# SEAME-pt/Team02-ObjectDetection

Hardware: NVIDIA B200
Metric: MobileNetV2UNet inference images/s (higher is better)
Workload: dtype bf16

## Files before the change

### include/b200seg.h

```cpp
#ifndef B200SEG_H_
#define B200SEG_H_

#include <stdint.h>

#ifdef __cplusplus
extern "C" {
#endif

typedef struct CUstream_st* b200seg_stream_t;

enum { B200SEG_F32 = 0, B200SEG_BF16 = 1 };
enum { B200SEG_ACT_NONE = 0, B200SEG_ACT_RELU = 1, B200SEG_ACT_RELU6 = 2 };

int b200seg_version(void);
const char* b200seg_last_error(void);
int b200seg_device_info(int* sm_count, int* cc);

int b200seg_conv3x3_smallcin(const void* x, int x_dtype, const float* w, const float* b, void* y,
                             int y_dtype, int B, int Cin, int H, int W, int Cout, int stride, int act,
                             b200seg_stream_t s);

int b200seg_stem_mb1_supported(int x_dtype, int H, int W, int Cstem, int Cout);
int b200seg_stem_mb1(const void* x, int x_dtype, const float* w_stem, const float* b_stem, const void* w_dw,
                     const float* b_dw, const void* w_pw, const float* b_pw, void* y, int B, int H, int W,
                     b200seg_stream_t s);

int b200seg_dwconv3x3(const void* x, const float* w, const float* b, void* y, int dtype, int B, int H,
                      int W, int C, int stride, int act, b200seg_stream_t s);

int b200seg_dwconv3x3_bf16w(const void* x, const void* w, const float* b, void* y, int B, int H, int W, int C, int stride,
                            int act, int variant, b200seg_stream_t s);

int b200seg_conv_tc(const void* x, const void* w, const float* b, const void* res, void* y, int B, int H,
                    int W, int Cin, int Cout, int taps, int act, int flags, b200seg_stream_t s);

int b200seg_conv_rs_supported(int H, int W, int Cin, int Cout);
int b200seg_conv_rs(const void* x, const void* w, const float* b, const void* res, void* y, int B, int H, int W, int Cin,
                    int Cout, int act, int flags, b200seg_stream_t s);

int b200seg_dwconv3x3_tc(const void* x, const void* wdiag, const float* b, void* y, int B, int H, int W,
                         int C, int stride, int act, int flags, b200seg_stream_t s);

int b200seg_conv_simt(const void* x, const float* w, const float* b, const void* res, void* y, int dtype,
                      int B, int H, int W, int Cin, int Cout, int taps, int act, b200seg_stream_t s);

int b200seg_upsample2x_concat(const void* skip, const void* x, void* y, int dtype, int B, int h, int w,
                              int Cs, int Cu, b200seg_stream_t s);

int b200seg_upsample2x_ac_nchw(const void* logits, int dtype, int ldc, void* out, int out_dtype, int B,
                               int h, int w, int C, b200seg_stream_t s);
int b200seg_upsample2x_ac_argmax(const void* logits, int dtype, int ldc, uint8_t* mask, int B, int h,
                                 int w, int C, b200seg_stream_t s);

int b200seg_mbconv(const void* x, const void* w_exp, const float* b_exp, const void* w_dw, const float* b_dw,
                   const void* w_proj, const float* b_proj, int residual, void* y, int B, int H, int W, int Cin,
                   int Ce, int Cout, int stride, int flags, b200seg_stream_t s);

int b200seg_tail_fused(const void* x, const void* w0, const float* b0, const void* w3, const float* b3, void* out,
                       int out_dtype, uint8_t* mask, int B, int h, int w, int C, b200seg_stream_t s);

int b200seg_nhwc_to_nchw(const void* x, int dtype, int ldc, void* out, int out_dtype, int B, int H, int W,
                         int C, b200seg_stream_t s);

int b200seg_maxpool2x2(const void* x, void* y, int dtype, int B, int H, int W, int C, b200seg_stream_t s);

int b200seg_softmax_ce(const float* logits, const int64_t* target, float* loss_sum, float* dlogits,
                       float grad_scale, const float* counts, int B, int C, int H, int W, b200seg_stream_t s);
int b200seg_scale_unless_one(float* x, long long n, const float* s, b200seg_stream_t st);
int b200seg_ce_count(const int64_t* target, float* counts, long long N, int C, long long ignore_index,
                     b200seg_stream_t s);

int b200seg_upsample2x_ac_generic(const void* logits, int dtype, int ldc, void* out, int out_dtype, uint8_t* mask, int B,
                                  int h, int w, int C, b200seg_stream_t s);
int b200seg_final_bwd_generic(const float* dout, void* dlogits, int dtype, int B, int h, int w, int C, int ldc,
                              b200seg_stream_t s);
int b200seg_nhwc_argmax(const void* x, int dtype, int ldc, uint8_t* mask, long long P, int C, b200seg_stream_t s);

int b200seg_bn_stats(const void* z, int dtype, long long P, int C, double* sum, double* sumsq, int nslot,
                     long long slot_stride, b200seg_stream_t s);
int b200seg_bn_finalize(const void* z, int dtype, const double* sum, const double* sumsq, int nslot,
                        long long slot_stride, long long n, const float* gamma,
                        const float* beta, float eps, float momentum, float* running_mean, float* running_var,
                        float* mean, float* invstd, float* scale, float* shift, int C, b200seg_stream_t s);
int b200seg_bn_apply(const void* z, const float* scale, const float* shift, const void* res, void* a, int dtype,
                     long long P, int C, int act, b200seg_stream_t s);
int b200seg_bn_finalize_apply(const void* z, const double* st_sums, int nslot, const float* gamma, const float* beta, float eps,
                              float momentum, float* running_mean, float* running_var, float* sv, const void* res, void* a,
                              int dtype, long long P, int C, int act, b200seg_stream_t s);
int b200seg_bn_bwd_reduce(const void* da, const void* z, const float* scale, const float* shift, const float* mean,
                          const float* invstd, int dtype, long long P, int C, int act, double* sg, double* sgx,
                          int nslot, long long slot_stride, b200seg_stream_t s);
int b200seg_bn_bwd_apply(const void* da, const void* z, const float* scale, const float* shift, const float* mean,
                         const float* invstd, const float* sg, const float* sgx, void* dz, int dtype, long long P,
                         int C, int act, b200seg_stream_t s);
int b200seg_bn_bwd_apply_slots(const void* da, const void* z, const float* sv, const double* red, int nslot, void* dz,
                               int dtype, long long P, int C, int act, b200seg_stream_t s);
int b200seg_bn_cluster_supported(int dtype, long long P, int C);
int b200seg_bn_cluster_bwd_supported(int dtype, long long P, int C);
int b200seg_bn_cluster_fwd(const void* z, long long P, int C, const float* gamma, const float* beta, float eps, float momentum,
                           float* running_mean, float* running_var, float* sv, const void* res, void* a, int act,
                           b200seg_stream_t s);
int b200seg_bn_cluster_bwd(const void* da, const void* z, const float* sv, long long P, int C, int act, double* red, void* dz,
                           b200seg_stream_t s);
int b200seg_act_bwd(const void* da, const void* a_out, void* dz, int dtype, long long N, int act, b200seg_stream_t s);
int b200seg_colsum(const void* x, int dtype, long long P, int C, double* out, int nslot, long long slot_stride,
                   b200seg_stream_t s);
int b200seg_f64_to_f32(const double* in, float* out, int n, int nslot, long long slot_stride, float scale,
                       b200seg_stream_t s);
int b200seg_conv_wgrad(const void* x, const void* dz, float* dw, int dtype, int B, int H, int W, int Cin, int Cout,
                       int taps, b200seg_stream_t s);
int b200seg_conv_wgrad_tc(const void* x, const void* dz, float* dw, int B, int H, int W, int Cin, int Cout, int taps,
                          b200seg_stream_t s);
int b200seg_dw_dgrad(const void* dz, const float* w, const void* acc_in, void* dx, int dtype, int B, int H, int W,
                     int C, int stride, b200seg_stream_t s);
int b200seg_dw_wgrad(const void* x, const void* dz, double* dw, int nslot, int dtype, int B, int H, int W, int C,
                     int stride, b200seg_stream_t s);
int b200seg_smallcin_wgrad(const void* x, int x_dtype, const void* dz, int dtype, float* dw, int B, int Cin, int H,
                           int W, int Cout, int stride, b200seg_stream_t s);
int b200seg_upcat_bwd(const void* dcat, const void* acc_skip, void* dskip, void* dx, int dtype, int B, int h, int w,
                      int Cs, int Cu, b200seg_stream_t s);
int b200seg_final_bwd(const float* dout, void* dlogits, int dtype, int B, int h, int w, int C, b200seg_stream_t s);
int b200seg_nchw_to_nhwc_pad(const float* x, void* y, int dtype, int B, int C, int H, int W, int ldc,
                             b200seg_stream_t s);
int b200seg_maxpool_bwd(const void* x, const void* dy, const void* acc_in, void* dx, int dtype, int B, int H, int W,
                        int C, b200seg_stream_t s);

int b200seg_adam_multi(const void* table, const int* chunk_tensor, const int* chunk_index, int n_chunks, float lr,
                       double one_minus_beta1, float beta2, double one_minus_beta2, float eps, float weight_decay,
                       double bias_corr1, double bias_corr2, b200seg_stream_t s);
int b200seg_adam_chunk(void);
int b200seg_pack_weights_multi(const void* table, const int* chunk_tensor, const int* chunk_index, int n_chunks,
                               b200seg_stream_t s);
int b200seg_pack_chunk(void);
int b200seg_fold_pack_eval_multi(const void* table, const int* chunk_tensor, const int* chunk_index, int n_chunks,
                                 b200seg_stream_t s);
int b200seg_fold_chunk(void);
int b200seg_grad_finalize_multi(const void* table, const int* chunk_tensor, const int* chunk_index, int n_chunks,
                                b200seg_stream_t s);
int b200seg_grad_chunk(void);

int b200seg_preprocess_u8(const uint8_t* frames, int B, int Hs, int Ws, void* out, int out_dtype, uint8_t* rgb, int H,
                          int W, float mean0, float mean1, float mean2, float std0, float std1, float std2,
                          b200seg_stream_t s);

int b200seg_remap_labels(const uint8_t* in, int64_t* out, const uint8_t* lut256, long long n, b200seg_stream_t s);

#ifdef __cplusplus
}
#endif
#endif
```

### team02-objectdetection_b200/b200seg/_cabi.py

```python
from __future__ import annotations

import ctypes as C
import os

_HERE = os.path.dirname(os.path.abspath(__file__))
LIB_PATH = os.path.join(_HERE, "libb200seg.so")

F32, BF16 = 0, 1
ACT_NONE, ACT_RELU, ACT_RELU6 = 0, 1, 2

_vp, _i, _f, _ll, _d = C.c_void_p, C.c_int, C.c_float, C.c_longlong, C.c_double

_PROTOS = {
    "b200seg_version": [],
    "b200seg_device_info": [C.POINTER(_i), C.POINTER(_i)],
    "b200seg_conv3x3_smallcin": [_vp, _i, _vp, _vp, _vp, _i, _i, _i, _i, _i, _i, _i, _i, _vp],
    "b200seg_stem_mb1_supported": [_i, _i, _i, _i, _i],
    "b200seg_stem_mb1": [_vp, _i, _vp, _vp, _vp, _vp, _vp, _vp, _vp, _i, _i, _i, _vp],
    "b200seg_dwconv3x3": [_vp, _vp, _vp, _vp, _i, _i, _i, _i, _i, _i, _i, _vp],
    "b200seg_dwconv3x3_bf16w": [_vp, _vp, _vp, _vp, _i, _i, _i, _i, _i, _i, _i, _vp],
    "b200seg_conv_tc": [_vp, _vp, _vp, _vp, _vp, _i, _i, _i, _i, _i, _i, _i, _i, _vp],
    "b200seg_conv_rs_supported": [_i, _i, _i, _i],
    "b200seg_conv_rs": [_vp, _vp, _vp, _vp, _vp, _i, _i, _i, _i, _i, _i, _i, _vp],
    "b200seg_dwconv3x3_tc": [_vp, _vp, _vp, _vp, _i, _i, _i, _i, _i, _i, _i, _vp],
    "b200seg_mbconv": [_vp, _vp, _vp, _vp, _vp, _vp, _vp, _i, _vp, _i, _i, _i, _i, _i, _i, _i, _i, _vp],
    "b200seg_conv_simt": [_vp, _vp, _vp, _vp, _vp, _i, _i, _i, _i, _i, _i, _i, _i, _vp],
    "b200seg_upsample2x_concat": [_vp, _vp, _vp, _i, _i, _i, _i, _i, _i, _vp],
    "b200seg_upsample2x_ac_nchw": [_vp, _i, _i, _vp, _i, _i, _i, _i, _i, _vp],
    "b200seg_upsample2x_ac_argmax": [_vp, _i, _i, _vp, _i, _i, _i, _i, _vp],
    "b200seg_tail_fused": [_vp, _vp, _vp, _vp, _vp, _vp, _i, _vp, _i, _i, _i, _i, _vp],
    "b200seg_nhwc_to_nchw": [_vp, _i, _i, _vp, _i, _i, _i, _i, _i, _vp],
    "b200seg_maxpool2x2": [_vp, _vp, _i, _i, _i, _i, _i, _vp],
    "b200seg_softmax_ce": [_vp, _vp, _vp, _vp, _f, _vp, _i, _i, _i, _i, _vp],
    "b200seg_scale_unless_one": [_vp, _ll, _vp, _vp],
    "b200seg_remap_labels": [_vp, _vp, _vp, _ll, _vp],
    "b200seg_ce_count": [_vp, _vp, _ll, _i, _ll, _vp],
    "b200seg_upsample2x_ac_generic": [_vp, _i, _i, _vp, _i, _vp, _i, _i, _i, _i, _vp],
    "b200seg_final_bwd_generic": [_vp, _vp, _i, _i, _i, _i, _i, _i, _vp],
    "b200seg_nhwc_argmax": [_vp, _i, _i, _vp, _ll, _i, _vp],
    "b200seg_bn_stats": [_vp, _i, _ll, _i, _vp, _vp, _i, _ll, _vp],
    "b200seg_bn_finalize": [_vp, _i, _vp, _vp, _i, _ll, _ll, _vp, _vp, _f, _f, _vp, _vp, _vp, _vp, _vp, _vp, _i, _vp],
    "b200seg_bn_apply": [_vp, _vp, _vp, _vp, _vp, _i, _ll, _i, _i, _vp],
    "b200seg_bn_bwd_reduce": [_vp, _vp, _vp, _vp, _vp, _vp, _i, _ll, _i, _i, _vp, _vp, _i, _ll, _vp],
    "b200seg_bn_cluster_supported": [_i, _ll, _i],
    "b200seg_bn_cluster_bwd_supported": [_i, _ll, _i],
    "b200seg_bn_cluster_fwd": [_vp, _ll, _i, _vp, _vp, _f, _f, _vp, _vp, _vp, _vp, _vp, _i, _vp],
    "b200seg_bn_cluster_bwd": [_vp, _vp, _vp, _ll, _i, _i, _vp, _vp, _vp],
    "b200seg_bn_bwd_apply": [_vp, _vp, _vp, _vp, _vp, _vp, _vp, _vp, _vp, _i, _ll, _i, _i, _vp],
    "b200seg_bn_bwd_apply_slots": [_vp, _vp, _vp, _vp, _i, _vp, _i, _ll, _i, _i, _vp],
    "b200seg_bn_finalize_apply": [_vp, _vp, _i, _vp, _vp, _f, _f, _vp, _vp, _vp, _vp, _vp, _i, _ll, _i, _i, _vp],
    "b200seg_act_bwd": [_vp, _vp, _vp, _i, _ll, _i, _vp],
    "b200seg_colsum": [_vp, _i, _ll, _i, _vp, _i, _ll, _vp],
    "b200seg_f64_to_f32": [_vp, _vp, _i, _i, _ll, _f, _vp],
    "b200seg_conv_wgrad": [_vp, _vp, _vp, _i, _i, _i, _i, _i, _i, _i, _vp],
    "b200seg_conv_wgrad_tc": [_vp, _vp, _vp, _i, _i, _i, _i, _i, _i, _vp],
    "b200seg_dw_dgrad": [_vp, _vp, _vp, _vp, _i, _i, _i, _i, _i, _i, _vp],
    "b200seg_dw_wgrad": [_vp, _vp, _vp, _i, _i, _i, _i, _i, _i, _i, _vp],
    "b200seg_smallcin_wgrad": [_vp, _i, _vp, _i, _vp, _i, _i, _i, _i, _i, _i, _vp],
    "b200seg_upcat_bwd": [_vp, _vp, _vp, _vp, _i, _i, _i, _i, _i, _i, _vp],
    "b200seg_final_bwd": [_vp, _vp, _i, _i, _i, _i, _i, _vp],
    "b200seg_nchw_to_nhwc_pad": [_vp, _vp, _i, _i, _i, _i, _i, _i, _vp],
    "b200seg_preprocess_u8": [_vp, _i, _i, _i, _vp, _i, _vp, _i, _i, _f, _f, _f, _f, _f, _f, _vp],
    "b200seg_adam_multi": [_vp, _vp, _vp, _i, _f, _d, _f, _d, _f, _f, _d, _d, _vp],
    "b200seg_adam_chunk": [],
    "b200seg_pack_weights_multi": [_vp, _vp, _vp, _i, _vp],
    "b200seg_pack_chunk": [],
    "b200seg_fold_pack_eval_multi": [_vp, _vp, _vp, _i, _vp],
    "b200seg_fold_chunk": [],
    "b200seg_grad_finalize_multi": [_vp, _vp, _vp, _i, _vp],
    "b200seg_grad_chunk": [],
    "b200seg_maxpool_bwd": [_vp, _vp, _vp, _vp, _i, _i, _i, _i, _i, _vp],
}
EXPORTS = sorted(list(_PROTOS) + ["b200seg_last_error"])


def _load():
    if not os.path.exists(LIB_PATH):
        raise ImportError(
            f"{LIB_PATH} not found: build it with `python team02-objectdetection_b200/build.py` "
            "(nvcc, sm_100a). b200seg has no CPU/eager fallback.")
    lib = C.CDLL(LIB_PATH)
    for name, args in _PROTOS.items():
        fn = getattr(lib, name)
        fn.argtypes = args
        fn.restype = _i
    lib.b200seg_last_error.argtypes = []
    lib.b200seg_last_error.restype = C.c_char_p
    return lib


lib = _load()


LAUNCHES = [0]


def check(rc: int, what: str = "") -> None:
    LAUNCHES[0] += 1
    if rc != 0:
        msg = lib.b200seg_last_error().decode("utf-8", "replace")
        raise RuntimeError(f"libb200seg {what} failed (rc={rc}): {msg}")


def ptr(t) -> int:
    return 0 if t is None else t.data_ptr()


def device_info():
    sm, cc = _i(0), _i(0)
    check(lib.b200seg_device_info(C.byref(sm), C.byref(cc)), "device_info")
    return sm.value, cc.value
```

### team02-objectdetection_b200/b200seg/ops.py

```python
from __future__ import annotations

from typing import Optional

import os

import torch

from . import _cabi
from ._cabi import ACT_NONE, ACT_RELU, ACT_RELU6, BF16, F32, check, lib, ptr

_DT = {torch.float32: F32, torch.bfloat16: BF16}


def _dt(t: torch.Tensor) -> int:
    try:
        return _DT[t.dtype]
    except KeyError:
        raise TypeError(f"b200seg supports float32 and bfloat16 activations, got {t.dtype}") from None


def _cuda(*ts):
    for t in ts:
        if t is None:
            continue
        if not t.is_cuda:
            raise RuntimeError("b200seg ops need CUDA tensors (no CPU fallback)")
        if not t.is_contiguous():
            raise RuntimeError("b200seg ops need contiguous tensors")


def _stream() -> int:
    return torch.cuda.current_stream().cuda_stream


_MUTATION_EPOCH = 0


def mutation_epoch() -> int:
    return _MUTATION_EPOCH


def bump_mutation_epoch() -> None:
    global _MUTATION_EPOCH
    _MUTATION_EPOCH += 1


def conv3x3_smallcin(x_nchw, w, b, stride: int, act: int, out_dtype, out=None):
    _cuda(x_nchw, w, b)
    B, Cin, H, W = x_nchw.shape
    Cout = w.shape[-1]
    Ho, Wo = (H - 1) // stride + 1, (W - 1) // stride + 1
    if out is None:
        out = torch.empty((B, Ho, Wo, Cout), device=x_nchw.device, dtype=out_dtype)
    check(lib.b200seg_conv3x3_smallcin(ptr(x_nchw), _dt(x_nchw), ptr(w), ptr(b), ptr(out), _dt(out), B, Cin, H, W,
                                       Cout, stride, act, _stream()), "conv3x3_smallcin")
    return out


def stem_mb1_supported(x_nchw, cstem: int, cout: int) -> bool:
    return bool(lib.b200seg_stem_mb1_supported(_dt(x_nchw), x_nchw.shape[2], x_nchw.shape[3], cstem, cout))


def stem_mb1(x_nchw, w_stem, b_stem, w_dw, b_dw, w_pw, b_pw, out=None):
    _cuda(x_nchw, w_stem, b_stem, w_dw, b_dw, w_pw, b_pw)
    B, C, H, W = x_nchw.shape
    if C != 3 or not x_nchw.is_contiguous():
        raise ValueError("stem_mb1 expects a contiguous NCHW tensor with 3 channels")
    if w_dw.dtype != torch.bfloat16 or w_pw.dtype != torch.bfloat16 or w_stem.dtype != torch.float32:
        raise TypeError("stem_mb1: w_stem f32, w_dw / w_pw bf16")
    if out is None:
        out = torch.empty((B, H // 2, W // 2, w_pw.shape[0]), device=x_nchw.device, dtype=torch.bfloat16)
    check(lib.b200seg_stem_mb1(ptr(x_nchw), _dt(x_nchw), ptr(w_stem), ptr(b_stem), ptr(w_dw), ptr(b_dw), ptr(w_pw), ptr(b_pw),
                               ptr(out), B, H, W, _stream()), "stem_mb1")
    return out


def dwconv3x3(x, w9c, b, stride: int, act: int, out=None):
    _cuda(x, w9c, b)
    B, H, W, Cc = x.shape
    Ho, Wo = (H - 1) // stride + 1, (W - 1) // stride + 1
    if out is None:
        out = torch.empty((B, Ho, Wo, Cc), device=x.device, dtype=x.dtype)
    check(lib.b200seg_dwconv3x3(ptr(x), ptr(w9c), ptr(b), ptr(out), _dt(x), B, H, W, Cc, stride, act, _stream()),
          "dwconv3x3")
    return out


def dwconv3x3_bf16w(x, w9c_bf16, b, stride: int, act: int, out=None, variant: int = 0):
    _cuda(x, w9c_bf16, b)
    if x.dtype != torch.bfloat16 or w9c_bf16.dtype != torch.bfloat16:
        raise TypeError("dwconv3x3_bf16w is bf16-only")
    B, H, W, Cc = x.shape
    if tuple(w9c_bf16.shape) != (9, Cc):
        raise ValueError(f"dwconv3x3_bf16w: taps {tuple(w9c_bf16.shape)} != (9, {Cc})")
    Ho, Wo = (H - 1) // stride + 1, (W - 1) // stride + 1
    if out is None:
        out = torch.empty((B, Ho, Wo, Cc), device=x.device, dtype=torch.bfloat16)
    check(lib.b200seg_dwconv3x3_bf16w(ptr(x), ptr(w9c_bf16), ptr(b), ptr(out), B, H, W, Cc, stride, act, variant, _stream()),
          "dwconv3x3_bf16w")
    return out


def pack_dw_diag(w9c: torch.Tensor) -> torch.Tensor:
    C = w9c.shape[1]
    out = torch.zeros(C, 9, 64, device=w9c.device, dtype=torch.bfloat16)
    idx = torch.arange(C, device=w9c.device)
    out[idx, :, idx % 64] = w9c.t().to(torch.bfloat16)
    return out.contiguous()


def dwconv3x3_tc(x, wdiag, b, stride: int, act: int, out=None, flags: int = 0):
    _cuda(x, wdiag, b)
    if x.dtype != torch.bfloat16 or wdiag.dtype != torch.bfloat16:
        raise TypeError("dwconv3x3_tc is bf16-only")
    B, H, W, Cc = x.shape
    if tuple(wdiag.shape) != (Cc, 9, 64):
        raise ValueError(f"dwconv3x3_tc: wdiag {tuple(wdiag.shape)} != ({Cc}, 9, 64)")
    Ho, Wo = (H - 1) // stride + 1, (W - 1) // stride + 1
    if out is None:
        out = torch.empty((B, Ho, Wo, Cc), device=x.device, dtype=torch.bfloat16)
    check(lib.b200seg_dwconv3x3_tc(ptr(x), ptr(wdiag), ptr(b), ptr(out), B, H, W, Cc, stride, act, flags, _stream()),
          "dwconv3x3_tc")
    return out


USE_CONV_RS = True
CONV_RS_FLAGS = 0


def conv_rs(x, w, b, act: int, res=None, out=None, flags: int = 0):
    _cuda(x, w, b, res)
    if x.dtype != torch.bfloat16 or w.dtype != torch.bfloat16:
        raise TypeError("conv_rs is bf16-only")
    B, H, W, Cin = x.shape
    Cout = w.shape[0]
    if w.shape[1] != 9 * Cin:
        raise ValueError(f"conv_rs: weight {tuple(w.shape)} does not match Cin={Cin}")
    if out is None:
        out = torch.empty((B, H, W, Cout), device=x.device, dtype=torch.bfloat16)
    check(lib.b200seg_conv_rs(ptr(x), ptr(w), ptr(b), ptr(res), ptr(out), B, H, W, Cin, Cout, act, flags, _stream()), "conv_rs")
    return out


def conv_tc(x, w, b, taps: int, act: int, res=None, out=None, flags: int = 0):
    _cuda(x, w, b, res)
    if x.dtype != torch.bfloat16 or w.dtype != torch.bfloat16:
        raise TypeError("conv_tc is bf16-only")
    B, H, W, Cin = x.shape
    Cout = w.shape[0]
    if w.shape[1] != taps * Cin:
        raise ValueError(f"conv_tc: weight {tuple(w.shape)} does not match taps={taps} Cin={Cin}")
    if (taps == 9 and USE_CONV_RS and flags == 0 and lib.b200seg_conv_rs_supported(H, W, Cin, Cout)
            and (Cout <= 32 or res is None)):
        return conv_rs(x, w, b, act, res, out, CONV_RS_FLAGS)
    if out is None:
        out = torch.empty((B, H, W, Cout), device=x.device, dtype=torch.bfloat16)
    check(lib.b200seg_conv_tc(ptr(x), ptr(w), ptr(b), ptr(res), ptr(out), B, H, W, Cin, Cout, taps, act, flags,
                              _stream()), "conv_tc")
    return out


def conv_simt(x, w, b, taps: int, act: int, res=None, out=None):
    _cuda(x, w, b, res)
    if w.dtype != torch.float32:
        raise TypeError("conv_simt weights are f32")
    B, H, W, Cin = x.shape
    Cout = w.shape[0]
    if w.shape[1] != taps * Cin:
        raise ValueError(f"conv_simt: weight {tuple(w.shape)} does not match taps={taps} Cin={Cin}")
    if out is None:
        out = torch.empty((B, H, W, Cout), device=x.device, dtype=x.dtype)
    check(lib.b200seg_conv_simt(ptr(x), ptr(w), ptr(b), ptr(res), ptr(out), _dt(x), B, H, W, Cin, Cout, taps, act,
                                _stream()), "conv_simt")
    return out


def pad_channels(t: torch.Tensor, mult: int) -> torch.Tensor:
    c = t.shape[-1]
    cp = (c + mult - 1) // mult * mult
    if cp == c:
        return t.contiguous()
    out = torch.zeros((*t.shape[:-1], cp), device=t.device, dtype=t.dtype)
    out[..., :c] = t
    return out


def mbconv(x, w_exp, b_exp, w_dw, b_dw, w_proj, b_proj, stride: int, residual: bool, out=None, flags: int = 0):
    _cuda(x, w_exp, b_exp, w_dw, b_dw, w_proj, b_proj)
    if x.dtype != torch.bfloat16 or w_exp.dtype != torch.bfloat16 or w_proj.dtype != torch.bfloat16 or w_dw.dtype != torch.bfloat16:
        raise TypeError("mbconv is bf16-only (activations, 1x1 weights and depthwise taps)")
    B, H, W, Cin = x.shape
    Ce, Cout = w_exp.shape[0], w_proj.shape[0]
    cep, cop = (Ce + 63) // 64 * 64, (Cout + 15) // 16 * 16
    if (tuple(w_exp.shape) != (Ce, Cin) or tuple(w_proj.shape) != (Cout, Ce) or tuple(w_dw.shape) != (9, cep)
            or b_exp.numel() != cep or b_dw.numel() != cep or b_proj.numel() != cop):
        raise ValueError(f"mbconv: operand shapes w_exp {tuple(w_exp.shape)} w_dw {tuple(w_dw.shape)} "
                         f"w_proj {tuple(w_proj.shape)} b {b_exp.numel()},{b_dw.numel()},{b_proj.numel()}")
    Ho, Wo = (H - 1) // stride + 1, (W - 1) // stride + 1
    if out is None:
        out = torch.empty((B, Ho, Wo, Cout), device=x.device, dtype=torch.bfloat16)
    check(lib.b200seg_mbconv(ptr(x), ptr(w_exp), ptr(b_exp), ptr(w_dw), ptr(b_dw), ptr(w_proj), ptr(b_proj),
                             1 if residual else 0, ptr(out), B, H, W, Cin, Ce, Cout, stride, flags, _stream()), "mbconv")
    return out


def upsample2x_concat(skip, x, out=None):
    _cuda(skip, x)
    B, h, w, Cu = x.shape
    Cs = skip.shape[3]
    if skip.shape[:3] != (B, 2 * h, 2 * w) or skip.dtype != x.dtype:
        raise ValueError(f"upsample2x_concat: skip {tuple(skip.shape)} vs x {tuple(x.shape)}")
    if out is None:
        out = torch.empty((B, 2 * h, 2 * w, Cs + Cu), device=x.device, dtype=x.dtype)
    check(lib.b200seg_upsample2x_concat(ptr(skip), ptr(x), ptr(out), _dt(x), B, h, w, Cs, Cu, _stream()),
          "upsample2x_concat")
    return out


def upsample2x_ac_nchw(logits, C: int, out_dtype, out=None):
    _cuda(logits)
    B, h, w, ldc = logits.shape
    if out is None:
        out = torch.empty((B, C, 2 * h, 2 * w), device=logits.device, dtype=out_dtype)
    if ldc != 16:
        check(lib.b200seg_upsample2x_ac_generic(ptr(logits), _dt(logits), ldc, ptr(out), _dt(out), None, B, h, w, C,
                                                _stream()), "upsample2x_ac_generic")
        return out
    check(lib.b200seg_upsample2x_ac_nchw(ptr(logits), _dt(logits), ldc, ptr(out), _dt(out), B, h, w, C, _stream()),
          "upsample2x_ac_nchw")
    return out


def upsample2x_ac_argmax(logits, C: int, out=None):
    _cuda(logits)
    B, h, w, ldc = logits.shape
    if out is None:
        out = torch.empty((B, 2 * h, 2 * w), device=logits.device, dtype=torch.uint8)
    if ldc != 16:
        check(lib.b200seg_upsample2x_ac_generic(ptr(logits), _dt(logits), ldc, None, F32, ptr(out), B, h, w, C,
                                                _stream()), "upsample2x_ac_generic")
        return out
    check(lib.b200seg_upsample2x_ac_argmax(ptr(logits), _dt(logits), ldc, ptr(out), B, h, w, C, _stream()),
          "upsample2x_ac_argmax")
    return out


def tail_fused(x, w0, b0, w3, b3, C: int, out_dtype=None, want_mask: bool = False, out=None):
    _cuda(x, w0, b0, w3, b3)
    B, h, w, cin = x.shape
    if (x.dtype != torch.bfloat16 or cin != 32 or tuple(w0.shape) != (16, 32) or tuple(w3.shape) != (16, 16)
            or w0.dtype != torch.bfloat16 or w3.dtype != torch.bfloat16 or b0.numel() < 16 or b3.numel() < 16 or not 1 <= C <= 16):
        raise ValueError("tail_fused: expects the MobileNetV2UNet tail (32 -> 16 -> C <= 16 channels, bf16)")
    if out is not None:
        want = (B, 2 * h, 2 * w) if want_mask else (B, C, 2 * h, 2 * w)
        if (tuple(out.shape) != want or out.dtype != (torch.uint8 if want_mask else out_dtype) or not out.is_contiguous()
                or out.device != x.device):
            raise ValueError(f"tail_fused: out must be a contiguous {want} tensor of the result dtype on {x.device}")
    if want_mask:
        if out is None:
            out = torch.empty((B, 2 * h, 2 * w), device=x.device, dtype=torch.uint8)
        check(lib.b200seg_tail_fused(ptr(x), ptr(w0), ptr(b0), ptr(w3), ptr(b3), None, F32, ptr(out), B, h, w, C, _stream()),
              "tail_fused")
    else:
        if out is None:
            out = torch.empty((B, C, 2 * h, 2 * w), device=x.device, dtype=out_dtype)
        check(lib.b200seg_tail_fused(ptr(x), ptr(w0), ptr(b0), ptr(w3), ptr(b3), ptr(out), _dt(out), None, B, h, w, C, _stream()),
              "tail_fused")
    return out


def nhwc_to_nchw(x, C: int, out_dtype, out=None):
    _cuda(x)
    B, H, W, ldc = x.shape
    if out is None:
        out = torch.empty((B, C, H, W), device=x.device, dtype=out_dtype)
    check(lib.b200seg_nhwc_to_nchw(ptr(x), _dt(x), ldc, ptr(out), _dt(out), B, H, W, C, _stream()), "nhwc_to_nchw")
    return out


def nhwc_argmax(x, C: int, out=None):
    _cuda(x)
    B, H, W, ldc = x.shape
    if out is None:
        out = torch.empty((B, H, W), device=x.device, dtype=torch.uint8)
    check(lib.b200seg_nhwc_argmax(ptr(x), _dt(x), ldc, ptr(out), B * H * W, C, _stream()), "nhwc_argmax")
    return out


def maxpool2x2(x, out=None):
    _cuda(x)
    B, H, W, Cc = x.shape
    if out is None:
        out = torch.empty((B, H // 2, W // 2, Cc), device=x.device, dtype=x.dtype)
    check(lib.b200seg_maxpool2x2(ptr(x), ptr(out), _dt(x), B, H, W, Cc, _stream()), "maxpool2x2")
    return out


IGNORE_INDEX = -100


def softmax_ce(logits, target, want_grad: bool = True, grad_scale: Optional[float] = None):
    _cuda(logits, target)
    if logits.dtype != torch.float32 or target.dtype != torch.int64:
        raise TypeError("softmax_ce expects f32 logits and int64 targets")
    B, Cc, H, W = logits.shape
    n = B * H * W
    acc = torch.zeros(3, device=logits.device, dtype=torch.float32)
    dl = torch.empty_like(logits) if want_grad else None
    if grad_scale is None:
        check(lib.b200seg_ce_count(ptr(target), ptr(acc[1:]), n, Cc, IGNORE_INDEX, _stream()), "ce_count")
        check(lib.b200seg_softmax_ce(ptr(logits), ptr(target), ptr(acc), ptr(dl), 1.0, ptr(acc[1:]), B, Cc, H, W, _stream()),
              "softmax_ce")
        loss = acc[0] / acc[1]
        return torch.where(acc[2] > 0, torch.full_like(loss, float("nan")), loss), dl
    check(lib.b200seg_softmax_ce(ptr(logits), ptr(target), ptr(acc), ptr(dl), grad_scale, None, B, Cc, H, W, _stream()),
          "softmax_ce")
    return acc[0] / n, dl


def scale_unless_one(x, s):
    _cuda(x, s)
    if x.dtype != torch.float32 or s.dtype != torch.float32 or not x.is_contiguous():
        raise TypeError("scale_unless_one: contiguous f32 tensors")
    check(lib.b200seg_scale_unless_one(ptr(x), x.numel(), ptr(s), _stream()), "scale_unless_one")
    return x


NSLOT = 16


class _ZeroPool:

    def __init__(self, dtype=torch.float64, chunk=1 << 20):
        self.buf, self.off, self.dtype, self.CHUNK = None, 0, dtype, chunk

    def reset(self):
        self.buf, self.off = None, 0

    def take(self, shape, device) -> torch.Tensor:
        n = 1
        for d in shape:
            n *= int(d)
        if self.buf is None or self.buf.device != device or self.off + n > self.buf.numel():
            self.buf = torch.zeros(max(n, self.CHUNK), device=device, dtype=self.dtype)
            self.off = 0
        t = self.buf[self.off:self.off + n].view(*shape)
        self.off += (n + 3) // 4 * 4
        return t


zero_pool = _ZeroPool()
zero_pool32 = _ZeroPool(torch.float32, 4 << 20)


def _P(t):
    return t.shape[0] * t.shape[1] * t.shape[2]


BN_CLUSTER = True


BN_FUSED_CONST = os.environ.get("B200SEG_BN_FUSED_CONST", "1") != "0"


def bn_train_forward(z, gamma, beta, running_mean, running_var, eps: float, momentum: float, act: int, res=None):
    _cuda(z, gamma, beta, running_mean, running_var, res)
    C, P = z.shape[-1], _P(z)
    if BN_CLUSTER and lib.b200seg_bn_cluster_supported(_dt(z), P, C):
        sv = torch.empty(4, C, device=z.device, dtype=torch.float32)
        a = torch.empty_like(z)
        check(lib.b200seg_bn_cluster_fwd(ptr(z), P, C, ptr(gamma), ptr(beta), eps, momentum, ptr(running_mean), ptr(running_var),
                                         ptr(sv), ptr(res), ptr(a), act, _stream()), "bn_cluster_fwd")
        return a, sv
    st = zero_pool.take((NSLOT, 2, C), z.device)
    check(lib.b200seg_bn_stats(ptr(z), _dt(z), P, C, ptr(st[0, 0]), ptr(st[0, 1]), NSLOT, 2 * C, _stream()), "bn_stats")
    sv = torch.empty(4, C, device=z.device, dtype=torch.float32)
    if BN_FUSED_CONST:
        a = torch.empty_like(z)
        check(lib.b200seg_bn_finalize_apply(ptr(z), ptr(st), NSLOT, ptr(gamma), ptr(beta), eps, momentum, ptr(running_mean),
                                            ptr(running_var), ptr(sv), ptr(res), ptr(a), _dt(z), P, C, act, _stream()),
              "bn_finalize_apply")
        return a, sv
    check(lib.b200seg_bn_finalize(ptr(z), _dt(z), ptr(st[0, 0]), ptr(st[0, 1]), NSLOT, 2 * C, P, ptr(gamma), ptr(beta), eps, momentum, ptr(running_mean),
                                  ptr(running_var), ptr(sv[0]), ptr(sv[1]), ptr(sv[2]), ptr(sv[3]), C, _stream()),
          "bn_finalize")
    a = torch.empty_like(z)
    check(lib.b200seg_bn_apply(ptr(z), ptr(sv[2]), ptr(sv[3]), ptr(res), ptr(a), _dt(z), P, C, act, _stream()), "bn_apply")
    return a, sv


def bn_train_backward(da, z, sv, act: int, red=None):
    _cuda(da, z, sv)
    C, P = z.shape[-1], _P(z)
    own_red = red is None
    if red is None:
        red = zero_pool.take((NSLOT, 2, C), z.device)
    if BN_CLUSTER and lib.b200seg_bn_cluster_bwd_supported(_dt(z), P, C):
        dz = torch.empty_like(z)
        check(lib.b200seg_bn_cluster_bwd(ptr(da), ptr(z), ptr(sv), P, C, act, ptr(red), ptr(dz), _stream()), "bn_cluster_bwd")
        if not own_red:
            return dz, None, None
        g32 = red[0].float()
        return dz, g32[1], g32[0]
    check(lib.b200seg_bn_bwd_reduce(ptr(da), ptr(z), ptr(sv[2]), ptr(sv[3]), ptr(sv[0]), ptr(sv[1]), _dt(z), P, C, act,
                                    ptr(red[0, 0]), ptr(red[0, 1]), NSLOT, 2 * C, _stream()), "bn_bwd_reduce")
    if BN_FUSED_CONST and not own_red:
        dz = torch.empty_like(z)
        check(lib.b200seg_bn_bwd_apply_slots(ptr(da), ptr(z), ptr(sv), ptr(red), NSLOT, ptr(dz), _dt(z), P, C, act, _stream()),
              "bn_bwd_apply_slots")
        return dz, None, None
    g32 = torch.empty(2, C, device=z.device, dtype=torch.float32)
    check(lib.b200seg_f64_to_f32(ptr(red), ptr(g32), 2 * C, NSLOT, 2 * C, 1.0, _stream()), "f64_to_f32")
    dz = torch.empty_like(z)
    check(lib.b200seg_bn_bwd_apply(ptr(da), ptr(z), ptr(sv[2]), ptr(sv[3]), ptr(sv[0]), ptr(sv[1]), ptr(g32[0]), ptr(g32[1]),
                                   ptr(dz), _dt(z), P, C, act, _stream()), "bn_bwd_apply")
    return dz, g32[1], g32[0]


def act_bwd(da, a_out, act: int):
    _cuda(da, a_out)
    dz = torch.empty_like(da)
    check(lib.b200seg_act_bwd(ptr(da), ptr(a_out), ptr(dz), _dt(da), da.numel(), act, _stream()), "act_bwd")
    return dz


def colsum(x, acc=None):
    _cuda(x)
    C = x.shape[-1]
    if acc is not None:
        check(lib.b200seg_colsum(ptr(x), _dt(x), _P(x), C, ptr(acc), NSLOT, C, _stream()), "colsum")
        return None
    acc = zero_pool.take((NSLOT, C), x.device)
    check(lib.b200seg_colsum(ptr(x), _dt(x), _P(x), C, ptr(acc), NSLOT, C, _stream()), "colsum")
    out = torch.empty(C, device=x.device, dtype=torch.float32)
    check(lib.b200seg_f64_to_f32(ptr(acc), ptr(out), C, NSLOT, C, 1.0, _stream()), "f64_to_f32")
    return out


def conv_wgrad(x, dz, taps: int, dw=None):
    _cuda(x, dz)
    B, H, W, Cin = x.shape
    Cout = dz.shape[-1]
    if dw is None:
        dw = zero_pool32.take((Cout, taps * Cin), x.device)
    check(lib.b200seg_conv_wgrad(ptr(x), ptr(dz), ptr(dw), _dt(x), B, H, W, Cin, Cout, taps, _stream()), "conv_wgrad")
    return dw


def conv_wgrad_tc(x, dz, taps: int, dw=None):
    _cuda(x, dz)
    if x.dtype != torch.bfloat16 or dz.dtype != torch.bfloat16:
        raise TypeError("conv_wgrad_tc is bf16-only")
    B, H, W, Cin = x.shape
    Cout = dz.shape[-1]
    if dw is None:
        dw = zero_pool32.take((Cout, taps * Cin), x.device)
    check(lib.b200seg_conv_wgrad_tc(ptr(x), ptr(dz), ptr(dw), B, H, W, Cin, Cout, taps, _stream()), "conv_wgrad_tc")
    return dw


def dw_dgrad(dz, w9c, in_shape, stride: int, acc=None):
    _cuda(dz, w9c, acc)
    B, H, W, Cc = in_shape
    dx = torch.empty(in_shape, device=dz.device, dtype=dz.dtype)
    check(lib.b200seg_dw_dgrad(ptr(dz), ptr(w9c), ptr(acc), ptr(dx), _dt(dz), B, H, W, Cc, stride, _stream()), "dw_dgrad")
    return dx


def dw_wgrad(x, dz, stride: int, acc=None):
    _cuda(x, dz)
    B, H, W, Cc = x.shape
    if acc is not None:
        check(lib.b200seg_dw_wgrad(ptr(x), ptr(dz), ptr(acc), NSLOT, _dt(x), B, H, W, Cc, stride, _stream()), "dw_wgrad")
        return None
    acc = zero_pool.take((NSLOT, 9, Cc), x.device)
    check(lib.b200seg_dw_wgrad(ptr(x), ptr(dz), ptr(acc), NSLOT, _dt(x), B, H, W, Cc, stride, _stream()), "dw_wgrad")
    out = torch.empty(9, Cc, device=x.device, dtype=torch.float32)
    check(lib.b200seg_f64_to_f32(ptr(acc), ptr(out), 9 * Cc, NSLOT, 9 * Cc, 1.0, _stream()), "f64_to_f32")
    return out


def smallcin_wgrad(x_nchw, dz, stride: int, dw=None):
    _cuda(x_nchw, dz)
    B, Cin, H, W = x_nchw.shape
    Cout = dz.shape[-1]
    if dw is None:
        dw = zero_pool32.take((3, 3, Cin, Cout), dz.device)
    check(lib.b200seg_smallcin_wgrad(ptr(x_nchw), _dt(x_nchw), ptr(dz), _dt(dz), ptr(dw), B, Cin, H, W, Cout, stride,
                                     _stream()), "smallcin_wgrad")
    return dw


def upcat_bwd(dcat, Cs: int, acc_skip=None):
    _cuda(dcat, acc_skip)
    B, H2, W2, Cc = dcat.shape
    h, w, Cu = H2 // 2, W2 // 2, Cc - Cs
    dskip = torch.empty(B, H2, W2, Cs, device=dcat.device, dtype=dcat.dtype)
    dx = torch.empty(B, h, w, Cu, device=dcat.device, dtype=dcat.dtype)
    check(lib.b200seg_upcat_bwd(ptr(dcat), ptr(acc_skip), ptr(dskip), ptr(dx), _dt(dcat), B, h, w, Cs, Cu, _stream()),
          "upcat_bwd")
    return dskip, dx


def final_bwd(dout_nchw, sdt, ldc: int = 16, out=None):
    _cuda(dout_nchw)
    if dout_nchw.dtype != torch.float32:
        raise TypeError("final_bwd expects f32 upstream gradients")
    B, Cc, H2, W2 = dout_nchw.shape
    dl = out if out is not None else torch.empty(B, H2 // 2, W2 // 2, ldc, device=dout_nchw.device, dtype=sdt)
    if tuple(dl.shape) != (B, H2 // 2, W2 // 2, ldc) or dl.dtype != sdt or not dl.is_contiguous():
        raise ValueError("final_bwd: bad output buffer")
    if ldc != 16:
        check(lib.b200seg_final_bwd_generic(ptr(dout_nchw), ptr(dl), _dt(dl), B, H2 // 2, W2 // 2, Cc, ldc, _stream()),
              "final_bwd_generic")
        return dl
    check(lib.b200seg_final_bwd(ptr(dout_nchw), ptr(dl), _dt(dl), B, H2 // 2, W2 // 2, Cc, _stream()), "final_bwd")
    return dl


def nchw_to_nhwc_pad(x_nchw, ldc: int, sdt, out=None):
    _cuda(x_nchw)
    B, Cc, H, W = x_nchw.shape
    y = out if out is not None else torch.empty(B, H, W, ldc, device=x_nchw.device, dtype=sdt)
    if tuple(y.shape) != (B, H, W, ldc) or y.dtype != sdt or not y.is_contiguous():
        raise ValueError("nchw_to_nhwc_pad: bad output buffer")
    check(lib.b200seg_nchw_to_nhwc_pad(ptr(x_nchw), ptr(y), _dt(y), B, Cc, H, W, ldc, _stream()), "nchw_to_nhwc_pad")
    return y


def maxpool_bwd(x, dy, acc=None):
    _cuda(x, dy, acc)
    B, H, W, Cc = x.shape
    dx = torch.empty_like(x)
    check(lib.b200seg_maxpool_bwd(ptr(x), ptr(dy), ptr(acc), ptr(dx), _dt(x), B, H, W, Cc, _stream()), "maxpool_bwd")
    return dx
```

### team02-objectdetection_b200/csrc/conv_rs.cu

```cuda
#include "common.cuh"

namespace b200 {

struct ConvRsArgs {
  const float* bias;
  const void* res;
  void* y;
  int Cin, Cout;
  int W, H, B;
  int BW, tiles_w;
  int k_chunks, stages;
  int act;
  long long total_rows;
};

constexpr int RS_THREADS = 192;
constexpr int RS_HALO_BYTES = 17 * 1024;

template <typename F>
__device__ __forceinline__ void rs_walk(long long g0, long long g1, int H, F&& f) {
  long long g = g0;
  while (g < g1) {
    const long long strip = g / H;
    const int ha = (int)(g - strip * H);
    const int hb = (int)min((long long)H, (long long)ha + (g1 - g));
    for (int r = ha - 1; r <= hb; ++r) f(strip, r, r >= 0 && r < H, r - 1 >= ha, r == ha - 1);
    g += hb - ha;
  }
}

template <int CN>
__global__ void __launch_bounds__(RS_THREADS, CN <= 32 ? 2 : 1)
conv_rs_kernel(const __grid_constant__ CUtensorMap tmA, const __grid_constant__ CUtensorMap tmB, const ConvRsArgs a) {
  extern __shared__ uint8_t smem_raw[];
  uint8_t* smem = smem_raw + ((1024u - (smem_u32(smem_raw) & 1023u)) & 1023u);
  const int warp = threadIdx.x >> 5, lane = threadIdx.x & 31;
  constexpr int NACC = 3 * CN;
  constexpr int B_TILE = NACC * 128;

  uint8_t* sA = smem;
  uint8_t* sB = sA + a.stages * RS_HALO_BYTES;
  float* sBias = reinterpret_cast<float*>(sB + a.k_chunks * 3 * B_TILE);
  uint64_t* full = reinterpret_cast<uint64_t*>(sBias + CN);
  uint64_t* empty = full + 8;
  uint64_t* acc_full = empty + 8;
  uint64_t* acc_empty = acc_full + 2;
  uint64_t* b_full = acc_empty + 2;
  uint32_t* tmem_slot = reinterpret_cast<uint32_t*>(b_full + 1);

  if (warp == 0 && lane == 0) {
    tma_prefetch_desc(&tmA);
    tma_prefetch_desc(&tmB);
    for (int i = 0; i < a.stages; ++i) { mbar_init(&full[i], 1); mbar_init(&empty[i], 1); }
    for (int i = 0; i < 2; ++i) { mbar_init(&acc_full[i], 1); mbar_init(&acc_empty[i], 128); }
    mbar_init(b_full, 1);
    fence_barrier_init();
  }
  for (int i = threadIdx.x; i < CN; i += RS_THREADS) sBias[i] = (a.bias && i < a.Cout) ? a.bias[i] : 0.f;
  constexpr uint32_t TMEM_COLS = 2 * NACC <= 32 ? 32 : 2 * NACC <= 64 ? 64 : 2 * NACC <= 128 ? 128 : 2 * NACC <= 256 ? 256 : 512;
  if (warp == 1) {
    tmem_alloc(tmem_slot, TMEM_COLS);
    tmem_relinquish();
  }
  tc_fence_before();
  __syncthreads();
  tc_fence_after();
  const uint32_t tmem_base = *tmem_slot;
  const long long g0 = a.total_rows * blockIdx.x / gridDim.x, g1 = a.total_rows * (blockIdx.x + 1) / gridDim.x;

  if (warp == 0) {
    if (lane == 0) {
      mbar_arrive_expect_tx(b_full, (uint32_t)(a.k_chunks * 3 * B_TILE));
      for (int c = 0; c < a.k_chunks; ++c)
        for (int kw = 0; kw < 3; ++kw)
          for (int kh = 0; kh < 3; ++kh)
            tma_load_3d(sB + (c * 3 + kw) * B_TILE + kh * CN * 128, &tmB, b_full, c * 64, kh * 3 + kw, 0);
    }
    int s = 0;
    uint32_t ph = 0;
    rs_walk(g0, g1, a.H, [&](long long strip, int r, bool valid, bool, bool) {
      if (!valid) return;
      const int w0 = (int)(strip % a.tiles_w) * a.BW, bb = (int)(strip / a.tiles_w);
      for (int c = 0; c < a.k_chunks; ++c) {
        mbar_wait(&empty[s], ph ^ 1u, 1);
        if (lane == 0) {
          mbar_arrive_expect_tx(&full[s], 130u * 128u);
          tma_load_4d(sA + s * RS_HALO_BYTES, &tmA, &full[s], c * 64, w0 - 1, r, bb);
        }
        __syncwarp();
        if (++s == a.stages) { s = 0; ph ^= 1u; }
      }
    });
  } else if (warp == 1) {
    const uint32_t idesc = umma_idesc_bf16(128, NACC);
    const uint32_t desc_hi = (uint32_t)(umma_desc_k128(0) >> 32);
    const uint32_t a_lo0 = (uint32_t)umma_desc_k128(smem_u32(sA));
    const uint32_t b_lo0 = (uint32_t)umma_desc_k128(smem_u32(sB));
    mbar_wait(b_full, 0, 5);
    int s = 0, nrow = 0;
    uint32_t ph = 0;
    rs_walk(g0, g1, a.H, [&](long long, int, bool valid, bool, bool) {
      if (!valid) return;
      const int ab = nrow & 1;
      const uint32_t aph = (uint32_t)(nrow >> 1) & 1u;
      ++nrow;
      mbar_wait(&acc_empty[ab], aph ^ 1u, 6);
      tc_fence_after();
      const uint32_t tacc = tmem_base + (uint32_t)(ab * NACC);
      uint32_t first = 0;
      for (int c = 0; c < a.k_chunks; ++c) {
        const int ksteps = (min(64, a.Cin - c * 64) + 15) >> 4;
        const uint32_t a_lo = a_lo0 + (uint32_t)s * (RS_HALO_BYTES >> 4);
        mbar_wait(&full[s], ph, 2);
        tc_fence_after();
        if (elect_one()) {
#pragma unroll
          for (int kw = 0; kw < 3; ++kw) {
            const uint32_t al = a_lo + (uint32_t)kw * 8u;
            const uint32_t bl = b_lo0 + (uint32_t)(c * 3 + kw) * (B_TILE >> 4);
#pragma unroll
            for (int k = 0; k < 4; ++k)
              if (k < ksteps) { umma_bf16_lohi(tacc, al + 2u * k, bl + 2u * k, desc_hi, idesc, first); first = 1u; }
          }
          umma_commit(&empty[s]);
          if (c == a.k_chunks - 1) umma_commit(&acc_full[ab]);
        }
        __syncwarp();
        if (++s == a.stages) { s = 0; ph ^= 1u; }
      }
    });
  } else {
    const int q = warp & 3;
    const int p = q * 32 + lane;
    const float act_lo = (a.act != B200SEG_ACT_NONE) ? 0.f : -INFINITY;
    const float act_hi = (a.act == B200SEG_ACT_RELU6) ? 6.f : INFINITY;
    const bool vec32 = (a.Cout & 15) == 0;
    float run0[CN], run1[CN];
    int nrow = 0;
    rs_walk(g0, g1, a.H, [&](long long strip, int r, bool valid, bool emit, bool new_run) {
      const int w0 = (int)(strip % a.tiles_w) * a.BW, bb = (int)(strip / a.tiles_w);
      if (new_run) {
#pragma unroll
        for (int i = 0; i < CN; ++i) { run0[i] = 0.f; run1[i] = 0.f; }
      }
      const bool px_ok = p < a.BW && w0 + p < a.W;
      const long long pix = ((long long)bb * a.H + (r - 1)) * a.W + (w0 + p);
      const __nv_bfloat16* rp = reinterpret_cast<const __nv_bfloat16*>(a.res) + pix * a.Cout;
      __nv_bfloat16* yp = reinterpret_cast<__nv_bfloat16*>(a.y) + pix * a.Cout;
      int ab = 0;
      if (valid) {
        ab = nrow & 1;
        const uint32_t aph = (uint32_t)(nrow >> 1) & 1u;
        ++nrow;
        mbar_wait(&acc_full[ab], aph, 3);
        tc_fence_after();
      }
      const uint32_t trow = tmem_base + ((uint32_t)(q * 32) << 16) + (uint32_t)(ab * NACC);
#pragma unroll
      for (int j = 0; j < CN / 16; ++j) {
        uint32_t d0[16], d1[16], d2[16];
        if (valid) {
          tmem_ld16(trow + (uint32_t)(16 * j), d0);
          tmem_ld16(trow + (uint32_t)(CN + 16 * j), d1);
          tmem_ld16(trow + (uint32_t)(2 * CN + 16 * j), d2);
          tmem_ld_wait();
        } else {
#pragma unroll
          for (int i = 0; i < 16; ++i) { d0[i] = 0u; d1[i] = 0u; d2[i] = 0u; }
        }
        float f[16];
#pragma unroll
        for (int i = 0; i < 16; ++i) {
          f[i] = run0[16 * j + i] + __uint_as_float(d2[i]);
          run0[16 * j + i] = run1[16 * j + i] + __uint_as_float(d1[i]);
          run1[16 * j + i] = __uint_as_float(d0[i]);
        }
        if (emit && px_ok && 16 * j < a.Cout) {
          const bool c_ok1 = 16 * j + 8 < a.Cout;
#pragma unroll
          for (int i = 0; i < 16; ++i) f[i] = fminf(fmaxf(f[i] + sBias[16 * j + i], act_lo), act_hi);
          if (a.res != nullptr) {
            const uint4 u0 = __ldg(reinterpret_cast<const uint4*>(rp + 16 * j));
            uint4 u1 = make_uint4(0, 0, 0, 0);
            if (c_ok1) u1 = __ldg(reinterpret_cast<const uint4*>(rp + 16 * j + 8));
            const uint32_t t[8] = {u0.x, u0.y, u0.z, u0.w, u1.x, u1.y, u1.z, u1.w};
#pragma unroll
            for (int i = 0; i < 8; ++i) { f[2 * i] += bf16lo(t[i]); f[2 * i + 1] += bf16hi(t[i]); }
          }
          uint32_t o[8];
#pragma unroll
          for (int i = 0; i < 8; ++i) o[i] = pack_bf16x2(f[2 * i], f[2 * i + 1]);
          if (vec32) {
            asm volatile("st.global.v8.b32 [%0], {%1,%2,%3,%4,%5,%6,%7,%8};" ::"l"(yp + 16 * j), "r"(o[0]), "r"(o[1]),
                         "r"(o[2]), "r"(o[3]), "r"(o[4]), "r"(o[5]), "r"(o[6]), "r"(o[7])
                         : "memory");
          } else {
            *reinterpret_cast<uint4*>(yp + 16 * j) = make_uint4(o[0], o[1], o[2], o[3]);
            if (c_ok1) *reinterpret_cast<uint4*>(yp + 16 * j + 8) = make_uint4(o[4], o[5], o[6], o[7]);
          }
        }
      }
      if (valid) {
        tc_fence_before();
        mbar_arrive(&acc_empty[ab]);
      }
    });
    tc_fence_before();
  }
  __syncthreads();
  if (warp == 1) {
    tc_fence_after();
    tmem_dealloc(tmem_base, TMEM_COLS);
  }
}

template <int CN>
static int launch_conv_rs(const CUtensorMap& tmA, const CUtensorMap& tmB, ConvRsArgs a, int flags, cudaStream_t stream) {
  const int b_all = a.k_chunks * 3 * (3 * CN * 128);
  const int fixed = b_all + CN * 4 + 256 + 1024 ;
  const int tmem_cols = 2 * 3 * CN <= 256 ? 256 : 512;
  int per_sm = (tmem_cols <= 256 && CN <= 32) ? 2 : 1;
  int stages = (227 * 1024 / per_sm - 1024 - fixed) / RS_HALO_BYTES;
  if (per_sm == 2 && stages < 2) { per_sm = 1; stages = (227 * 1024 - 1024 - fixed) / RS_HALO_BYTES; }
  if ((flags >> 20) & 3) { per_sm = (flags >> 20) & 3; stages = (227 * 1024 / per_sm - 1024 - fixed) / RS_HALO_BYTES; }
  if (stages > 8) stages = 8;
  if ((flags >> 16) & 0xf) stages = min(stages, (flags >> 16) & 0xf);
  B200_REQUIRE(stages >= 2, "conv_rs: weights do not leave room for a load ring (Cin=%d Cout=%d)", a.Cin, a.Cout);
  a.stages = stages;
  const int smem = fixed + stages * RS_HALO_BYTES;
  static bool attr = false;
  if (!attr) {
    cudaError_t e = cudaFuncSetAttribute(conv_rs_kernel<CN>, cudaFuncAttributeMaxDynamicSharedMemorySize, 227 * 1024);
    if (e != cudaSuccess) return set_error((int)e, "conv_rs: cudaFuncSetAttribute: %s", cudaGetErrorString(e));
    attr = true;
  }
  long long grid = (long long)sm_count() * per_sm;
  if ((flags >> 8) & 0xff) grid = (long long)((flags >> 8) & 0xff) * 4;
  if (grid > a.total_rows) grid = a.total_rows;
  conv_rs_kernel<CN><<<(unsigned)grid, RS_THREADS, (size_t)smem, stream>>>(tmA, tmB, a);
  return check_launch("conv_rs");
}

}

using namespace b200;

extern "C" int b200seg_conv_rs_supported(int H, int W, int Cin, int Cout) {
  const int cn = (Cout + 15) & ~15;
  const int k_chunks = (Cin + 63) / 64;
  return (cn == 16 || cn == 32 || cn == 80) && W >= 96 && H >= 3 && Cin % 8 == 0 && Cout % 8 == 0 &&
         k_chunks * 3 * (3 * cn * 128) <= 120 * 1024;
}

extern "C" int b200seg_conv_rs(const void* x, const void* w, const float* bias, const void* res, void* y, int B, int H,
                               int W, int Cin, int Cout, int act, int flags, b200seg_stream_t s) {
  B200_REQUIRE(x && w && y && B > 0, "conv_rs: bad arguments");
  B200_REQUIRE(b200seg_conv_rs_supported(H, W, Cin, Cout), "conv_rs: unsupported shape H=%d W=%d Cin=%d Cout=%d", H, W, Cin, Cout);
  ConvRsArgs a;
  a.bias = bias; a.res = res; a.y = y;
  a.Cin = Cin; a.Cout = Cout; a.W = W; a.H = H; a.B = B;
  a.BW = W < 128 ? W : 128;
  a.tiles_w = (W + a.BW - 1) / a.BW;
  a.k_chunks = (Cin + 63) / 64;
  a.act = act;
  a.total_rows = (long long)B * a.tiles_w * H;
  const int cn = (Cout + 15) & ~15;
  CUtensorMap tmA, tmB;
  {
    uint64_t dims[4] = {(uint64_t)Cin, (uint64_t)W, (uint64_t)H, (uint64_t)B};
    uint64_t str[3] = {(uint64_t)Cin * 2, (uint64_t)Cin * 2 * W, (uint64_t)Cin * 2 * W * H};
    uint32_t box[4] = {64, 130, 1, 1};
    int rc = make_tmap_bf16(&tmA, x, 4, dims, str, box, 1, nullptr);
    if (rc) return rc;
  }
  {
    uint64_t dims[3] = {(uint64_t)Cin, 9, (uint64_t)Cout};
    uint64_t str[2] = {(uint64_t)Cin * 2, (uint64_t)Cin * 2 * 9};
    uint32_t box[3] = {64, 1, (uint32_t)cn};
    int rc = make_tmap_bf16(&tmB, w, 3, dims, str, box, 1, nullptr);
    if (rc) return rc;
  }
  if (cn == 16) return launch_conv_rs<16>(tmA, tmB, a, flags, (cudaStream_t)s);
  if (cn == 80) return launch_conv_rs<80>(tmA, tmB, a, flags, (cudaStream_t)s);
  return launch_conv_rs<32>(tmA, tmB, a, flags, (cudaStream_t)s);
}
```

Before: 34540.

## Split conv_rs output channels across CTA groups and add a Cout=64 variant

Extends the row-streaming 3x3 tensor-core conv kernel so that layers with Cout up to 64 can run either as one CN=64 tile or as two CTA groups, each computing a 32-channel output slice. Each group offsets its bias, weight TMA coordinate and output pointer by co0, and the row ranges are divided among grid/groups CTAs. This moves more 3x3 convs in the UNet decoder off the generic conv_tc path onto the halo-streaming kernel. In exchange, the split path loads each input halo twice, once per group. A new check enforces that the TMEM budget per SM is not exceeded.

```diff
diff --git a/include/b200seg.h b/include/b200seg.h
--- a/include/b200seg.h
+++ b/include/b200seg.h
@@ -35,6 +35,7 @@
                     int W, int Cin, int Cout, int taps, int act, int flags, b200seg_stream_t s);
 
 int b200seg_conv_rs_supported(int H, int W, int Cin, int Cout);
+int b200seg_conv_rs_groups(int H, int W, int Cin, int Cout);
 int b200seg_conv_rs(const void* x, const void* w, const float* b, const void* res, void* y, int B, int H, int W, int Cin,
                     int Cout, int act, int flags, b200seg_stream_t s);
 
diff --git a/team02-objectdetection_b200/b200seg/_cabi.py b/team02-objectdetection_b200/b200seg/_cabi.py
--- a/team02-objectdetection_b200/b200seg/_cabi.py
+++ b/team02-objectdetection_b200/b200seg/_cabi.py
@@ -21,6 +21,7 @@
     "b200seg_dwconv3x3_bf16w": [_vp, _vp, _vp, _vp, _i, _i, _i, _i, _i, _i, _i, _vp],
     "b200seg_conv_tc": [_vp, _vp, _vp, _vp, _vp, _i, _i, _i, _i, _i, _i, _i, _i, _vp],
     "b200seg_conv_rs_supported": [_i, _i, _i, _i],
+    "b200seg_conv_rs_groups": [_i, _i, _i, _i],
     "b200seg_conv_rs": [_vp, _vp, _vp, _vp, _vp, _i, _i, _i, _i, _i, _i, _i, _vp],
     "b200seg_dwconv3x3_tc": [_vp, _vp, _vp, _vp, _i, _i, _i, _i, _i, _i, _i, _vp],
     "b200seg_mbconv": [_vp, _vp, _vp, _vp, _vp, _vp, _vp, _i, _vp, _i, _i, _i, _i, _i, _i, _i, _i, _vp],
diff --git a/team02-objectdetection_b200/b200seg/ops.py b/team02-objectdetection_b200/b200seg/ops.py
--- a/team02-objectdetection_b200/b200seg/ops.py
+++ b/team02-objectdetection_b200/b200seg/ops.py
@@ -150,7 +150,7 @@
     Cout = w.shape[0]
     if w.shape[1] != taps * Cin:
         raise ValueError(f"conv_tc: weight {tuple(w.shape)} does not match taps={taps} Cin={Cin}")
-    if (taps == 9 and USE_CONV_RS and flags == 0 and lib.b200seg_conv_rs_supported(H, W, Cin, Cout)
+    if (taps == 9 and USE_CONV_RS and flags == 0 and lib.b200seg_conv_rs_groups(H, W, Cin, Cout)
             and (Cout <= 32 or res is None)):
         return conv_rs(x, w, b, act, res, out, CONV_RS_FLAGS)
     if out is None:
diff --git a/team02-objectdetection_b200/csrc/conv_rs.cu b/team02-objectdetection_b200/csrc/conv_rs.cu
--- a/team02-objectdetection_b200/csrc/conv_rs.cu
+++ b/team02-objectdetection_b200/csrc/conv_rs.cu
@@ -11,6 +11,7 @@
   int BW, tiles_w;
   int k_chunks, stages;
   int act;
+  int groups;
   long long total_rows;
 };
 
@@ -56,7 +57,8 @@
     mbar_init(b_full, 1);
     fence_barrier_init();
   }
-  for (int i = threadIdx.x; i < CN; i += RS_THREADS) sBias[i] = (a.bias && i < a.Cout) ? a.bias[i] : 0.f;
+  const int co0 = CN == 32 ? (int)(blockIdx.x % a.groups) * CN : 0;
+  for (int i = threadIdx.x; i < CN; i += RS_THREADS) sBias[i] = (a.bias && co0 + i < a.Cout) ? a.bias[co0 + i] : 0.f;
   constexpr uint32_t TMEM_COLS = 2 * NACC <= 32 ? 32 : 2 * NACC <= 64 ? 64 : 2 * NACC <= 128 ? 128 : 2 * NACC <= 256 ? 256 : 512;
   if (warp == 1) {
     tmem_alloc(tmem_slot, TMEM_COLS);
@@ -66,7 +68,8 @@
   __syncthreads();
   tc_fence_after();
   const uint32_t tmem_base = *tmem_slot;
-  const long long g0 = a.total_rows * blockIdx.x / gridDim.x, g1 = a.total_rows * (blockIdx.x + 1) / gridDim.x;
+  const long long ranges = gridDim.x / a.groups, rng = blockIdx.x / a.groups;
+  const long long g0 = a.total_rows * rng / ranges, g1 = a.total_rows * (rng + 1) / ranges;
 
   if (warp == 0) {
     if (lane == 0) {
@@ -74,7 +77,7 @@
       for (int c = 0; c < a.k_chunks; ++c)
         for (int kw = 0; kw < 3; ++kw)
           for (int kh = 0; kh < 3; ++kh)
-            tma_load_3d(sB + (c * 3 + kw) * B_TILE + kh * CN * 128, &tmB, b_full, c * 64, kh * 3 + kw, 0);
+            tma_load_3d(sB + (c * 3 + kw) * B_TILE + kh * CN * 128, &tmB, b_full, c * 64, kh * 3 + kw, co0);
     }
     int s = 0;
     uint32_t ph = 0;
@@ -145,8 +148,8 @@
       }
       const bool px_ok = p < a.BW && w0 + p < a.W;
       const long long pix = ((long long)bb * a.H + (r - 1)) * a.W + (w0 + p);
-      const __nv_bfloat16* rp = reinterpret_cast<const __nv_bfloat16*>(a.res) + pix * a.Cout;
-      __nv_bfloat16* yp = reinterpret_cast<__nv_bfloat16*>(a.y) + pix * a.Cout;
+      const __nv_bfloat16* rp = reinterpret_cast<const __nv_bfloat16*>(a.res) + pix * a.Cout + co0;
+      __nv_bfloat16* yp = reinterpret_cast<__nv_bfloat16*>(a.y) + pix * a.Cout + co0;
       int ab = 0;
       if (valid) {
         ab = nrow & 1;
@@ -175,8 +178,8 @@
           run0[16 * j + i] = run1[16 * j + i] + __uint_as_float(d1[i]);
           run1[16 * j + i] = __uint_as_float(d0[i]);
         }
-        if (emit && px_ok && 16 * j < a.Cout) {
-          const bool c_ok1 = 16 * j + 8 < a.Cout;
+        if (emit && px_ok && co0 + 16 * j < a.Cout) {
+          const bool c_ok1 = co0 + 16 * j + 8 < a.Cout;
 #pragma unroll
           for (int i = 0; i < 16; ++i) f[i] = fminf(fmaxf(f[i] + sBias[16 * j + i], act_lo), act_hi);
           if (a.res != nullptr) {
@@ -226,6 +229,7 @@
   if (stages > 8) stages = 8;
   if ((flags >> 16) & 0xf) stages = min(stages, (flags >> 16) & 0xf);
   B200_REQUIRE(stages >= 2, "conv_rs: weights do not leave room for a load ring (Cin=%d Cout=%d)", a.Cin, a.Cout);
+  B200_REQUIRE(per_sm * tmem_cols <= 512, "conv_rs: %d CTAs per SM need %d TMEM columns", per_sm, per_sm * tmem_cols);
   a.stages = stages;
   const int smem = fixed + stages * RS_HALO_BYTES;
   static bool attr = false;
@@ -236,26 +240,38 @@
   }
   long long grid = (long long)sm_count() * per_sm;
   if ((flags >> 8) & 0xff) grid = (long long)((flags >> 8) & 0xff) * 4;
-  if (grid > a.total_rows) grid = a.total_rows;
+  if (grid > a.total_rows * a.groups) grid = a.total_rows * a.groups;
+  grid -= grid % a.groups;
   conv_rs_kernel<CN><<<(unsigned)grid, RS_THREADS, (size_t)smem, stream>>>(tmA, tmB, a);
   return check_launch("conv_rs");
 }
 
+static int rs_group_cn(int H, int W, int Cin, int Cout, int groups) {
+  if (groups < 1) return 0;
+  const int cn = ((Cout + groups - 1) / groups + 15) & ~15;
+  const int k_chunks = (Cin + 63) / 64;
+  const bool variant = groups == 1 ? (cn == 16 || cn == 32 || cn == 64 || cn == 80) : (groups == 2 && cn == 32 && Cout > 32);
+  return (variant && W >= 96 && H >= 3 && Cin % 8 == 0 && Cout % 8 == 0 && k_chunks * 3 * (3 * cn * 128) <= 120 * 1024) ? cn : 0;
+}
+
 }
 
 using namespace b200;
 
-extern "C" int b200seg_conv_rs_supported(int H, int W, int Cin, int Cout) {
-  const int cn = (Cout + 15) & ~15;
-  const int k_chunks = (Cin + 63) / 64;
-  return (cn == 16 || cn == 32 || cn == 80) && W >= 96 && H >= 3 && Cin % 8 == 0 && Cout % 8 == 0 &&
-         k_chunks * 3 * (3 * cn * 128) <= 120 * 1024;
+extern "C" int b200seg_conv_rs_supported(int H, int W, int Cin, int Cout) { return rs_group_cn(H, W, Cin, Cout, 1) != 0; }
+
+extern "C" int b200seg_conv_rs_groups(int H, int W, int Cin, int Cout) {
+  for (int g = 1; g <= 2; ++g)
+    if (rs_group_cn(H, W, Cin, Cout, g)) return g;
+  return 0;
 }
 
 extern "C" int b200seg_conv_rs(const void* x, const void* w, const float* bias, const void* res, void* y, int B, int H,
                                int W, int Cin, int Cout, int act, int flags, b200seg_stream_t s) {
   B200_REQUIRE(x && w && y && B > 0, "conv_rs: bad arguments");
-  B200_REQUIRE(b200seg_conv_rs_supported(H, W, Cin, Cout), "conv_rs: unsupported shape H=%d W=%d Cin=%d Cout=%d", H, W, Cin, Cout);
+  const int groups = ((flags >> 22) & 3) ? ((flags >> 22) & 3) : b200seg_conv_rs_groups(H, W, Cin, Cout);
+  const int cn = rs_group_cn(H, W, Cin, Cout, groups);
+  B200_REQUIRE(cn, "conv_rs: unsupported shape H=%d W=%d Cin=%d Cout=%d (groups=%d)", H, W, Cin, Cout, groups);
   ConvRsArgs a;
   a.bias = bias; a.res = res; a.y = y;
   a.Cin = Cin; a.Cout = Cout; a.W = W; a.H = H; a.B = B;
@@ -263,8 +279,8 @@
   a.tiles_w = (W + a.BW - 1) / a.BW;
   a.k_chunks = (Cin + 63) / 64;
   a.act = act;
+  a.groups = groups;
   a.total_rows = (long long)B * a.tiles_w * H;
-  const int cn = (Cout + 15) & ~15;
   CUtensorMap tmA, tmB;
   {
     uint64_t dims[4] = {(uint64_t)Cin, (uint64_t)W, (uint64_t)H, (uint64_t)B};
@@ -281,6 +297,7 @@
     if (rc) return rc;
   }
   if (cn == 16) return launch_conv_rs<16>(tmA, tmB, a, flags, (cudaStream_t)s);
+  if (cn == 64) return launch_conv_rs<64>(tmA, tmB, a, flags, (cudaStream_t)s);
   if (cn == 80) return launch_conv_rs<80>(tmA, tmB, a, flags, (cudaStream_t)s);
   return launch_conv_rs<32>(tmA, tmB, a, flags, (cudaStream_t)s);
 }
```

Result: faster. 35390 (median of 6 runs) (+2.5%).
